# lukedan/libfluid

Hardware: AMD Instinct MI355X
Metric: particle_steps_per_sec (higher is better)
Workload: dtype f32

## Files before the change

### libfluid_amd/csrc/common.h

```cpp
#pragma once

#include <hip/hip_runtime.h>
#include <stdint.h>

#include <string>
#include <vector>

#include "../../include/libfluid_amd.h"
#include "slots.h"

hipError_t lfa_pool_malloc(void **p, size_t bytes);
hipError_t lfa_pool_free(void *p);
void lfa_pool_nosync_begin();
void lfa_pool_nosync_end();
template <typename T> inline hipError_t lfa_hip_malloc(T **p, size_t bytes) { return lfa_pool_malloc((void **)p, bytes); }
#define hipMalloc(p, n) lfa_hip_malloc((p), (n))
#define hipFree(p) lfa_pool_free((void *)(p))
struct lfa_stream_set;
lfa_stream_set *lfa_pool_take_set(int device);
void lfa_pool_park_set(lfa_stream_set *q);

#define LFA_TILE 8
#define LFA_TILE_CELLS 512
#define LFA_HALO 10
// ... 102 lines not shown
	float *uo = nullptr, *vo = nullptr, *wo = nullptr;
	uint8_t *ctype = nullptr, *solid = nullptr;
	uint32_t *cell_count = nullptr;
	uint32_t *fine_start = nullptr;
	float *stage = nullptr;
	size_t stage_tiles = 0;
	float *acc = nullptr;
	double bg[3] = {0, 0, 0};
	bool grid_valid = false;

	uint8_t *abits = nullptr;
	void *vp = nullptr, *vr = nullptr, *vz = nullptr, *vs = nullptr, *vpre = nullptr, *vq = nullptr;
	struct lfa_mg *mg = nullptr;
	int *nbr_table = nullptr;
	void *vs2 = nullptr;
	size_t vec_elem = 0;
	double *partials = nullptr;
	int *pcg_state = nullptr;
	double *pcg_hist = nullptr;
	int *level_tiles = nullptr;
	std::vector<int> level_offsets;
	GridDims g1{};
	size_t ncp1 = 0;
	float *c_diag = nullptr, *c_w[3] = {nullptr, nullptr, nullptr};
	uint8_t *c_unk = nullptr;
	void *c_pre = nullptr, *c_r = nullptr, *c_x = nullptr, *c_r2 = nullptr, *c_x2 = nullptr, *a2inv = nullptr;
	void *c_as = nullptr;
	int *slot_l1 = nullptr, *l1_tiles = nullptr, *l1_l2 = nullptr;
	int n_l1tiles = 0, n2 = 0, a2cap = 0;
	size_t coarse_elem = 0;
	double a_scale = 0.0, sys_dt = -1.0;
	uint64_t n_unknowns = 0;
	bool system_valid = false, unknown_count_valid = false;
	double last_residual = 0.0;
	uint64_t last_iters = 0;
	uint64_t stat_launches_iter = 0, stat_transport_iter = 0, stat_transport_solve = 0, stat_mg_levels = 0, stat_mg_first_co = 0;
	bool pcg_poisoned = false;
	bool last_rhs_zero = false;
	bool co_disabled = false;
	uint64_t stat_co_aborts = 0, stat_co_reason = 0;
	bool gate_counted = false;
	uint32_t *tile_epoch = nullptr;
	uint8_t *tile_closed = nullptr;
	uint32_t solve_epoch = 0;
	uint32_t pressure_epoch = 0;
	bool warm_started = false;
	uint32_t *vc_src = nullptr;
	size_t vc_extent = 0;
	bool vc_pending = false;
	uint64_t stat_p2g_deferred = 0;
	bool vmax2_valid = false;
	float *c_home = nullptr;
	size_t c_home_cap = 0;
	bool c_home_valid = false;
	bool vc_with_c = false;
	uint8_t *tile_clear = nullptr;
	unsigned clear_epoch = 0;
	unsigned solid_epoch = 1;

	struct SourceHost {
		std::vector<int32_t> xyz;
		double vel[3];
		uint64_t root;
		bool active, coerce;
		bool operator==(const SourceHost &o) const {
			return xyz == o.xyz && vel[0] == o.vel[0] && vel[1] == o.vel[1] && vel[2] == o.vel[2] && root == o.root &&
// ... 263 lines not shown
		v[k] = i < n ? p[i] : -INFINITY;
	}
	double a = -INFINITY;
#pragma unroll
	for (int k = 0; k < 8; ++k) {
		nan |= v[k] != v[k];
		a = v[k] > a ? v[k] : a;
	}
	for (int i = (int)threadIdx.x + 2048; i < n; i += 256) {
		const double x = p[i];
		nan |= x != x;
		a = x > a ? x : a;
	}
	return a;
}
template <typename T> __device__ inline T wave_sum(T v) {
#pragma unroll
	for (int o = 32; o > 0; o >>= 1) v += __shfl_xor(v, o, 64);
	return v;
}
template <typename T> __device__ inline T wave_max(T v) {
#pragma unroll
	for (int o = 32; o > 0; o >>= 1) {
		T other = __shfl_xor(v, o, 64);
		v = other > v ? other : v;
	}
	return v;
}

int lfa_exclusive_scan_u32(lfa_sim *s, const uint32_t *in, uint32_t *out, size_t n, uint32_t *total_dev);
int lfa_scan_total(lfa_sim *s, const uint32_t *in, uint32_t *out, size_t n, uint32_t *total_dev, int slot, size_t *total);

int lfa_particles_alloc(lfa_sim *s, size_t n);
int lfa_hash_particles_impl(lfa_sim *s, bool counts_done);
int lfa_particles_materialize(lfa_sim *s);
int lfa_c_home_restore(lfa_sim *s);
int lfa_c_home_ensure(lfa_sim *s, size_t n);
int lfa_ensure_io(lfa_sim *s, size_t bytes);
int lfa_slab_download_slots(lfa_sim *s, const uint32_t **slot);
int lfa_sample_velocity_launch(lfa_sim *s, hipStream_t stream, const double *xyz, size_t n, const uint32_t *tile_rule, int z_lo, int z_hi,
                               double *velocity, uint8_t *types, uint32_t *counts_dev);
int lfa_sample_refresh(lfa_sim *s, const char *who, size_t room_bytes, const uint32_t **tile_rule, void **room, int *z_lo, int *z_hi);
int lfa_pcg_alloc(lfa_sim *s);
int lfa_number_unknowns(lfa_sim *s);

__host__ __device__ inline int lfa_stage_index(int hx, int hy, int hz) {
	return (unsigned)(hx - 1) < 8u ? (hx - 1) + 8 * (hy + 10 * hz) : 800 + (hx ? 100 : 0) + hy + 10 * hz;
}
__host__ __device__ inline int lfa_stage_source(int o) {
	if (o < 800) return 1 + (o & 7) + 10 * (o >> 3);
	const int q = o - 800, pl = q >= 100 ? 1 : 0, r = q - 100 * pl;
	return 9 * pl + 10 * r;
}

struct lfa_dist {
	int rank = 0, nranks = 1;
	int device_share = 1;
	int exchange(lfa_sim *s, const void *send_lo, size_t n_send_lo, void *recv_lo, size_t n_recv_lo, const void *send_hi,
	             size_t n_send_hi, void *recv_hi, size_t n_recv_hi) {
		++calls;
		return exchange_impl(s, send_lo, n_send_lo, recv_lo, n_recv_lo, send_hi, n_send_hi, recv_hi, n_recv_hi);
	}
	int allreduce(lfa_sim *s, double *dev, int count, bool is_max) {
		++calls;
		return allreduce_impl(s, dev, count, is_max);
	}
	int allreduce_buf(lfa_sim *s, void *dev, size_t count, int dtype, bool is_max) {
// ... 44 lines not shown
```

### libfluid_amd/csrc/core.hip

```cpp
#include <math.h>

#include <algorithm>
#include <stdarg.h>
#include <stdio.h>
#include <string.h>

#include <mutex>

#include "common.h"
#include "pcg.h"
#include "stream_set.h"

static thread_local std::string g_create_error;

int lfa_fail(lfa_sim *s, int code, const char *fmt, ...) {
	char buf[512];
	va_list ap;
	va_start(ap, fmt);
	vsnprintf(buf, sizeof buf, fmt, ap);
	va_end(ap);
	if (s) s->err = buf;
	else g_create_error = buf;
	return code;
}
// ... 910 lines not shown
	pos_store(dst.pos, d, key, me.t[0], me.t[1], me.t[2]);
	bkey[d] = key;
	dst.id[d] = src.id[i];
	from[d] = (uint32_t)i;
}
__global__ void k_c_to_home(size_t n, ParticleSoA p, float *home, size_t stride) {
	size_t i = (size_t)blockIdx.x * blockDim.x + threadIdx.x;
	if (i >= n || p.pos[i].key == 0xFFFFFFFFu) return;
	const size_t j = p.id[i];
#pragma unroll
	for (int k = 0; k < 9; ++k) home[k * stride + j] = p.c[k][i];
}
__global__ void k_c_from_home(size_t n, ParticleSoA p, const float *home, size_t stride) {
	size_t i = (size_t)blockIdx.x * blockDim.x + threadIdx.x;
	if (i >= n || p.pos[i].key == 0xFFFFFFFFu) return;
	const size_t j = p.id[i];
#pragma unroll
	for (int k = 0; k < 9; ++k) p.c[k][i] = home[k * stride + j];
}
__global__ void k_gather_vc(size_t n, ParticleSoA old, ParticleSoA cur, const uint32_t *from, int with_c) {
	size_t d = (size_t)blockIdx.x * blockDim.x + threadIdx.x;
	if (d >= n) return;
	const uint32_t i = from[d];
#pragma unroll
	for (int k = 0; k < 3; ++k) cur.v[k][d] = old.v[k][i];
	if (with_c) {
#pragma unroll
		for (int k = 0; k < 9; ++k) cur.c[k][d] = old.c[k][i];
	}
}

#define CC_UNROLL 16
__global__ void __launch_bounds__(256)
k_cell_count(const int *dtiles, int n_dtiles, const uint32_t *key, const uint32_t *tile_start, uint32_t *cell_count) {
	__shared__ uint32_t cnt[LFA_TILE_CELLS];
	for (int slot = blockIdx.x; slot < n_dtiles; slot += gridDim.x) {
		int tile = dtiles[slot];
		cnt[threadIdx.x] = 0;
		cnt[threadIdx.x + 256] = 0;
		__syncthreads();
		uint32_t b = tile_start[tile], e = tile_start[tile + 1];
		for (uint32_t base = b + threadIdx.x; base - threadIdx.x < e; base += 256 * CC_UNROLL) {
			uint32_t k[CC_UNROLL];
#pragma unroll
			for (int q = 0; q < CC_UNROLL; ++q) {
				const uint32_t i = base + 256 * q;
				k[q] = key[i < e ? i : e - 1];
			}
#pragma unroll
			for (int q = 0; q < CC_UNROLL; ++q)
				if (base + 256 * q < e) atomicAdd(&cnt[k[q] & 511], 1u);
		}
		__syncthreads();
		cell_count[(size_t)tile * LFA_TILE_CELLS + threadIdx.x] = cnt[threadIdx.x];
		cell_count[(size_t)tile * LFA_TILE_CELLS + 256 + threadIdx.x] = cnt[threadIdx.x + 256];
		__syncthreads();
	}
}

__global__ void k_compact_range(const uint32_t *flag, const uint32_t *scan, int *list, int *slot_of, int lo, int hi,
                                int slot_base) {
	int t = lo + blockIdx.x * blockDim.x + threadIdx.x;
	if (t >= hi) return;
	if (flag[t]) {
		list[scan[t]] = t;
		if (slot_of) slot_of[t] = slot_base + (int)scan[t];
	} else if (slot_of) {
		slot_of[t] = -1;
	}
}
__global__ void k_fill_i32(int *p, int n, int v) {
	int i = blockIdx.x * blockDim.x + threadIdx.x;
	if (i < n) p[i] = v;
}
__global__ void k_gather_u32(const uint32_t *src, const int *idx, int n, uint32_t *dst) {
	int i = threadIdx.x;
	if (i < n) dst[i] = src[idx[i]];
}

__global__ void k_dilate_slots(const int *tile_pslot, uint32_t *flag, GridDims g) {
	const int t = blockIdx.x * blockDim.x + threadIdx.x;
	if (t >= g.nt || tile_pslot[t] < 0) return;
	int tx, ty, tz;
	tile_coords(g, t, tx, ty, tz);
	for (int o = 0; o < 27; ++o) {
		const int x = tx + o % 3 - 1, y = ty + (o / 3) % 3 - 1, z = tz + o / 9 - 1;
		if ((unsigned)x < (unsigned)g.ntx && (unsigned)y < (unsigned)g.nty && (unsigned)z < (unsigned)g.ntz)
			flag[x + g.ntx * (y + g.nty * z)] = 1u;
// ... 27 lines not shown
		const hipError_t e = hipStreamSynchronize(s->stream);
		if (e != hipSuccess) return fail(e, "hipStreamSynchronize");
		LFA_HIP(s, hipFree(s->c_home));
	}
	s->c_home = nh;
	s->c_home_cap = cap;
	return LFA_OK;
}
int lfa_c_home_restore(lfa_sim *s) {
	if (!s->c_home_valid) return LFA_OK;
	s->c_home_valid = false;
	const size_t n = s->binned ? s->np_live : s->np;
	if (!n) return LFA_OK;
	hipLaunchKernelGGL(k_c_from_home, dim3((unsigned)((n + 255) / 256)), dim3(256), 0, s->stream, n, s->pb[s->cur], (const float *)s->c_home,
	                   s->c_home_cap);
	LFA_LAUNCH_CHECK(s);
	return LFA_OK;
}

int lfa_particles_materialize(lfa_sim *s) {
	if (!s->vc_pending) return LFA_OK;
	LFA_TRY(lfa_corr_commit(s));
	s->vc_pending = false;
	LFA_HIP(s, hipSetDevice(s->device));
	const size_t n = s->np_live;
	if (!n) return LFA_OK;
	hipLaunchKernelGGL(k_gather_vc, dim3((unsigned)((n + 255) / 256)), dim3(256), 0, s->stream, n, s->pb[s->cur ^ 1], s->pb[s->cur],
	                   (const uint32_t *)s->vc_src, s->vc_with_c ? 1 : 0);
	LFA_LAUNCH_CHECK(s);
	return LFA_OK;
}

extern "C" int lfa_hash_particles(lfa_sim *s) { return lfa_hash_particles_impl(s, false); }
int lfa_hash_particles_impl(lfa_sim *s, bool counts_done) {
	if (!s) return LFA_E_INVALID;
	LFA_HIP(s, hipSetDevice(s->device));
	LFA_TRY(lfa_corr_commit(s));
	LFA_TRY(lfa_particles_materialize(s));
	const GridDims &g = s->g;
	const int nt = g.nt, L = g.ntx * g.nty;
	const size_t n = s->binned ? s->np_live : s->np;
	ParticleSoA &src = s->pb[s->cur], &dst = s->pb[s->cur ^ 1];
	const int own_lo = s->slab_lo * L, own_hi = s->slab_hi * L;
	const int all_lo = lfa_has_lo(s) ? own_lo - L : own_lo, all_hi = lfa_has_hi(s) ? own_hi + L : own_hi;

	if (!counts_done) {
		LFA_HIP(s, hipMemsetAsync(s->tile_count, 0, (size_t)(nt + 1) * 4, s->stream));
		if (n) {
			hipLaunchKernelGGL(k_tile_count, dim3((unsigned)((n + 256 * TC_CHUNKS - 1) / (256 * TC_CHUNKS))), dim3(256), 0, s->stream, (const PosRec *)src.pos, n,
			                   s->tile_count, s->rank);
			LFA_LAUNCH_CHECK(s);
		}
	}
	LFA_TRY(lfa_exclusive_scan_u32(s, s->tile_count, s->tile_start, (size_t)nt + 1, nullptr));
	LFA_HIP(s, hipMemcpyAsync(s->h_pinned + LFA_PIN_NP_LIVE, s->tile_start + nt, 4, hipMemcpyDeviceToHost, s->stream));

	hipLaunchKernelGGL(k_tile_flags, dim3((nt + 255) / 256), dim3(256), 0, s->stream, s->tile_count, s->tile_flag, nt);
	LFA_LAUNCH_CHECK(s);
	LFA_TRY(lfa_dist_exchange_tile_layers_u32(s, s->tile_flag));
	hipLaunchKernelGGL(k_fill_i32, dim3((nt + 255) / 256), dim3(256), 0, s->stream, s->tile_pslot, nt, -1);
	LFA_LAUNCH_CHECK(s);
	const bool one_sync = !s->dist;
	if (one_sync) {
		uint32_t *tot = (uint32_t *)s->pcg_state + LFA_DW_N_PTILES;
		LFA_TRY(compact_tiles_async(s, s->tile_flag, 0, nt, s->ptiles_all, s->tile_pslot, tot));
		LFA_HIP(s, hipMemsetAsync(s->tile_flag, 0, (size_t)(nt + 1) * 4, s->stream));
		hipLaunchKernelGGL(k_dilate_slots, dim3((nt + 255) / 256), dim3(256), 0, s->stream, (const int *)s->tile_pslot, s->tile_flag, g);
// ... 42 lines not shown
		s->n_ghost_lo = s->p_off;
		s->n_ghost_hi = s->n_ptiles_all - vals[3];
		s->ptiles = s->ptiles_all + s->p_off;
		s->n_dtiles = (int)h[LFA_SLAB_N_DTILES];
		for (int w = 0; w < 4; ++w) s->n_halo[w] = (int)h[LFA_SLAB_N_HALO + w];
	}
	s->np_live = s->h_pinned[LFA_PIN_NP_LIVE];
	if (s->dist) s->np = s->np_live;
	s->holes = false;
	s->n_arrivals = 0;
	s->move_pending = false;
	if (n) {
		const dim3 sgrid((unsigned)((n + 255) / 256));
		const bool home = s->prm.simulation_method != LFA_APIC;
		if (home && !s->c_home_valid) {
			LFA_TRY(lfa_c_home_ensure(s, s->dist ? std::max<size_t>(s->pcap, (size_t)s->next_global_id) : s->pcap));
			hipLaunchKernelGGL(k_c_to_home, sgrid, dim3(256), 0, s->stream, n, src, s->c_home, s->c_home_cap);
			LFA_LAUNCH_CHECK(s);
			s->c_home_valid = true;
		} else if (!home && s->c_home_valid) {
			LFA_TRY(lfa_c_home_restore(s));
		}
		hipLaunchKernelGGL(k_tile_scatter, sgrid, dim3(256), 0, s->stream, n, src, dst, s->rank, s->tile_start, s->tile_count,
		                   s->binned ? 0 : 1, s->vc_src, s->bkey);
		LFA_LAUNCH_CHECK(s);
		s->cur ^= 1;
		s->vc_pending = true;
		s->vc_extent = n;
		s->vc_with_c = !home;
	}
	if (s->n_dtiles) {
		int grid = s->n_dtiles < 8192 ? s->n_dtiles : 8192;
		hipLaunchKernelGGL(k_cell_count, dim3(grid), dim3(256), 0, s->stream, s->dtiles, s->n_dtiles,
		                   (const uint32_t *)s->bkey, s->tile_start, s->cell_count);
		LFA_LAUNCH_CHECK(s);
	}
	s->binned = true;
	s->system_valid = false;
	s->unknown_count_valid = false;
	return LFA_OK;
}

int lfa_dist_build_halo_lists(lfa_sim *s, const uint32_t *flag, int *lists, int n[4]) {
	const int L = s->g.ntx * s->g.nty;
	const int lo[4] = {s->slab_lo * L, (s->slab_hi - 1) * L, (s->slab_lo - 1) * L, s->slab_hi * L};
	const bool on[4] = {lfa_has_lo(s), lfa_has_hi(s), lfa_has_lo(s), lfa_has_hi(s)};
	uint32_t *tot = (uint32_t *)s->pcg_state + LFA_DW_SLAB + LFA_SLAB_N_HALO;
	LFA_HIP(s, hipMemsetAsync(tot, 0, 16, s->stream));
	for (int w = 0; w < 4; ++w)
		if (on[w]) LFA_TRY(compact_tiles_async(s, flag, lo[w], lo[w] + L, lists + (size_t)w * L, nullptr, tot + w));
	LFA_HIP(s, hipMemcpyAsync(s->h_pinned + LFA_PIN_SLAB + LFA_SLAB_N_HALO, tot, 16, hipMemcpyDeviceToHost, s->stream));
	LFA_HIP(s, hipStreamSynchronize(s->stream));
	for (int w = 0; w < 4; ++w) n[w] = (int)s->h_pinned[LFA_PIN_SLAB + LFA_SLAB_N_HALO + w];
	return LFA_OK;
}

__global__ void k_raw_unknown_flags(GridDims g, size_t nc, const uint32_t *cell_count, const uint32_t *tile_flag,
                                    uint32_t *flag, int z0, int z1) {
	size_t r = (size_t)blockIdx.x * blockDim.x + threadIdx.x;
	if (r >= nc) return;
	int x = (int)(r % g.nx), y = (int)((r / g.nx) % g.ny), z = (int)(r / ((size_t)g.nx * g.ny));
	uint32_t b = blocked_index(g, x, y, z);
	flag[r] = (z >= z0 && z < z1 && tile_flag[b >> 9] && cell_count[b] > 0) ? 1u : 0u;
}

int lfa_number_unknowns(lfa_sim *s) {
	if (s->unknown_count_valid) return LFA_OK;
	if (!s->binned) return lfa_fail(s, LFA_E_INVALID, "call lfa_hash_particles first");
	if (!s->raw_scan) LFA_HIP(s, hipMalloc(&s->raw_scan, (s->nc + 1) * 4));
// ... 243 lines not shown
```

### libfluid_amd/csrc/grid_ops.hip

```cpp
#include "common.h"
#include "pcg.h"

namespace {

struct GridView {
	GridDims g;
	const uint8_t *ctype, *solid;
	const uint32_t *cell_count, *tile_flag;
};
__device__ inline bool is_unknown_at(const GridView &gv, int x, int y, int z) {
	if (!in_grid(gv.g, x, y, z)) return false;
	uint32_t b = blocked_index(gv.g, x, y, z);
	return gv.tile_flag[b >> 9] && gv.cell_count[b] > 0;
}

#define HT_UNKNOWN 8
__device__ inline void stage_halo_types(const GridView &gv, int tx, int ty, int tz, uint8_t *H) {
	for (int i = threadIdx.x; i < LFA_HALO_CELLS; i += 256) {
		const int x = 8 * tx + i % 10 - 1, y = 8 * ty + (i / 10) % 10 - 1, z = 8 * tz + i / 100 - 1;
		uint8_t t = CT_SOLID;
		if (in_grid(gv.g, x, y, z)) {
			const uint32_t b = blocked_index(gv.g, x, y, z);
			if (gv.tile_flag[b >> 9]) t = (uint8_t)((gv.ctype[b] & 7) | (gv.cell_count[b] > 0 ? HT_UNKNOWN : 0));
			else t = gv.solid[b] ? CT_SOLID : CT_AIR;
// ... 447 lines not shown
		const float v2 = g2p_particle<METHOD>(
		    p, i, pold, (METHOD == LFA_FLIP_BLEND && from) ? from[i] : i, gp,
		    [&](int b0, int b1, int b2) { return make_int3(cx + b0, cy + b1, cz + b2); },
		    [&](int field, int comp, int3 c, int k) { return clamped_sample(g, F[field], comp, c.x + (k & 1), c.y + ((k >> 1) & 1), c.z + (k >> 2)); });
		vmax2 = fmaxf(vmax2, v2);
	}
	vmax2 = wave_max(vmax2);
	if ((threadIdx.x & 63) == 0 && vmax2 > 0.0f) atomicMax(vmax2_bits, __float_as_uint(vmax2));
}
}

static int grid_blocks(int n) { return n < 16384 ? (n > 0 ? n : 1) : 16384; }

int lfa_dist_refresh_grid(lfa_sim *s, bool with_topology) {
	if (!s->dist) return LFA_OK;
	void *f[9];
	int e[9], n = 0;
	f[n] = s->u; e[n++] = 4;
	f[n] = s->v; e[n++] = 4;
	f[n] = s->w; e[n++] = 4;
	if (with_topology) {
		f[n] = s->ctype; e[n++] = 1;
		f[n] = s->cell_count; e[n++] = 4;
		if (s->prm.simulation_method == LFA_FLIP_BLEND && s->uo) {
			f[n] = s->uo; e[n++] = 4;
			f[n] = s->vo; e[n++] = 4;
			f[n] = s->wo; e[n++] = 4;
		}
	}
	return lfa_dist_exchange_fields(s, n, f, e);
}
static GridView make_view(lfa_sim *s) { return GridView{s->g, s->ctype, s->solid, s->cell_count, s->tile_flag}; }

int lfa_build_rhs(lfa_sim *s, double dt) {
	if (!s->binned) return lfa_fail(s, LFA_E_INVALID, "lfa_build_system: call lfa_hash_particles first");
	LFA_TRY(lfa_pcg_alloc(s));
	LFA_TRY(lfa_dist_refresh_grid(s, true));
	s->a_scale = dt / (s->prm.density * s->prm.cell_size * s->prm.cell_size);
	s->sys_dt = dt;
	if (!s->n_ptiles) return LFA_OK;
	GridView gv = make_view(s);
	if (!s->tile_closed) {
		LFA_HIP(s, hipMalloc(&s->tile_closed, (size_t)s->g.nt));
		LFA_HIP(s, hipMemsetAsync(s->tile_closed, 0, (size_t)s->g.nt, s->stream));
	}
	hipLaunchKernelGGL(k_abits, dim3(grid_blocks(s->n_ptiles)), dim3(256), 0, s->stream, s->ptiles, s->n_ptiles, gv,
	                   s->abits, s->tile_closed);
	LFA_LAUNCH_CHECK(s);
	const int G = pcg_grid_uncapped(s->n_ptiles);
	const float inv_h = (float)(1.0 / s->prm.cell_size);
	if (!s->tile_epoch) {
		LFA_HIP(s, hipMalloc(&s->tile_epoch, (size_t)s->g.nt * 4));
		LFA_HIP(s, hipMemsetAsync(s->tile_epoch, 0, (size_t)s->g.nt * 4, s->stream));
	}
	s->warm_started = s->prm.pcg_warm_start && s->prm.precond != LFA_PRECOND_MIC0_EXACT && !s->dist && s->pressure_epoch == s->solve_epoch &&
	                  s->solve_epoch != 0;
	const uint32_t keep_epoch = s->warm_started ? s->solve_epoch : 0u;
	++s->solve_epoch;
	if (s->solve_epoch == 0) s->solve_epoch = 1;
	if (s->prm.pcg_dtype == LFA_PCG_F64)
		hipLaunchKernelGGL(k_rhs<double>, dim3(G), dim3(256), 0, s->stream, s->ptiles, s->n_ptiles, gv, s->u, s->v, s->w,
		                   (double *)s->vr, (double *)s->vp, inv_h, s->partials + PART_B2, s->tile_epoch, keep_epoch, s->solve_epoch);
	else
		hipLaunchKernelGGL(k_rhs<float>, dim3(G), dim3(256), 0, s->stream, s->ptiles, s->n_ptiles, gv, s->u, s->v, s->w,
		                   (float *)s->vr, (float *)s->vp, inv_h, s->partials + PART_B2, s->tile_epoch, keep_epoch, s->solve_epoch);
	LFA_LAUNCH_CHECK(s);
	return LFA_OK;
}

extern "C" int lfa_apply_pressure(lfa_sim *s, double dt) {
	if (!s) return LFA_E_INVALID;
	if (!s->binned || !s->vp) return lfa_fail(s, LFA_E_INVALID, "lfa_apply_pressure: no pressure on the device");
	LFA_HIP(s, hipSetDevice(s->device));
	if (s->dist) LFA_TRY(lfa_dist_exchange_slices(s, s->vp, s->prm.pcg_dtype == LFA_PCG_F64 ? 8 : 4));
	if (!s->n_dtiles) return LFA_OK;
	const float coeff = (float)(dt / (s->prm.density * s->prm.cell_size));
	GridView gv = make_view(s);
	dim3 grid(grid_blocks(s->n_dtiles));
	if (s->prm.pcg_dtype == LFA_PCG_F64)
		hipLaunchKernelGGL(k_apply_pressure<double>, grid, dim3(256), 0, s->stream, s->dtiles, s->n_dtiles, gv, s->u, s->v,
		                   s->w, (const double *)s->vp, coeff);
// ... 93 lines not shown
```

### libfluid_amd/csrc/mg.hip

```cpp
#include <mutex>

#include "pcg.h"

#include <limits.h>
#include <math.h>
#include <stdio.h>
#include <stdlib.h>

#include <algorithm>
#include <vector>

#define MG_MAX_LEVELS 12
#define MG_NBR_STRIDE 8
#ifndef MG_INNER_SWEEPS
#define MG_INNER_SWEEPS 2
#endif
#define MG_OMEGA 1.15

struct lfa_mg_level {
	GridDims g{};
	size_t ncp = 0;
	int n_tiles = 0;
	int *tiles = nullptr;
	int *nbr = nullptr;
// ... 2269 lines not shown
	}
	size_t wgs;
	LFA_TRY(mg_co_capacity<real>(s, false, 0, &wgs));
	auto fits = [&](int first, bool tg) {
		const int nlev = last - first + 1;
		if (nlev > MG_CO_MAX_LEVELS || mg_co_capacity<real>(s, tg, nlev, &wgs) != LFA_OK) return false;
		const size_t share = s->dist ? (size_t)std::max(1, s->dist->device_share) : 1;
		return M.lv[first].n_tiles <= MG_CO_MAX_TILES && (size_t)M.lv[first].n_tiles * share <= wgs;
	};
	auto first_inside = [&](bool tg) {
		int tl = last;
		while (tl > 1 && tl - 1 >= D && fits(tl - 1, tg)) --tl;
		return std::max(tl, std::max(D, 1));
	};
	bool tagged = sizeof(real) == 4 && !s->knobs.mg_no_tagged;
	int tail = first_inside(tagged);
	if (tagged) {
		for (int l = tail; l <= last && tagged; ++l) tagged = mg_ensure_xq(s, M.lv[l], 3);
		if (!tagged) tail = first_inside(false);
	}
	P.tail = tail;
	P.tagged = tagged;
	const bool shared_gpu = s->dist && s->dist->device_share > 1;
	if (tagged && !shared_gpu && tail - 1 >= std::max(D, 1) && M.lv[tail - 1].n_tiles > 0 && !s->knobs.mg_no_top &&
	    M.lv[tail - 1].n_tiles <= MG_TOP_MAX_TILES && mg_ensure_xq(s, M.lv[tail - 1], 1))
		P.top = tail - 1;
	return LFA_OK;
}

static int mg_plan(lfa_sim *s);

template <typename real> static int mg_setup_t(lfa_sim *s) {
	if (!s->mg) s->mg = new lfa_mg();
	MgSetup U;
	LFA_TRY(mg_setup_levels<real>(s, U));
	if (U.D) LFA_TRY(mg_setup_host_lists(s, U));
	else LFA_TRY(mg_setup_device_lists<real>(s, U));
	LFA_TRY(mg_setup_operators<real>(s, U));
	LFA_TRY(mg_setup_exchange_abits(s, U));
	return mg_plan(s);
}

int lfa_mg_setup(lfa_sim *s) {
	return s->prm.pcg_dtype == LFA_PCG_F64 ? mg_setup_t<double>(s) : mg_setup_t<float>(s);
}

template <typename real> static MgLv<real> mg_lv(const lfa_sim *s, int l) {
	const lfa_mg_level &L = s->mg->lv[l];
	return MgLv<real>{L.tiles, L.nbr, L.n_tiles, L.g, l == 0 ? (const uint8_t *)s->abits : (const uint8_t *)L.abits,
	                  l == 0 ? (real *)s->vr : (real *)L.b, l == 0 ? (real *)s->vq : (real *)L.x, l == 0 ? (real *)s->vz : (real *)L.y};
}

template <typename real> static int mg_launch_coarse(lfa_sim *s, int top, void (*co_kernel)(MgCo<real>, const int *)) {
	lfa_mg &M = *s->mg;
	const MgPlan &P = M.plan;
	const int last = P.last, tail = P.tail;
	const int *st = (const int *)s->pcg_state;
	if (P.persist) {
		MgCo<real> C;
		C.first = tail;
		C.last = last;
		C.nsw = MG_COARSEST_SWEEPS;
		C.inner = MG_INNER_SWEEPS;
		for (int l = tail; l <= last; ++l) {
			C.lv[l] = mg_lv<real>(s, l);
			C.ready[l] = M.lv[l].ready;
// ... 295 lines not shown
```

### libfluid_amd/csrc/p2g.hip

```cpp
#include "common.h"

namespace {

__device__ inline void axis_bf(float t, bool own, int &b, float &f) {
	if (own) {
		b = t >= 1.0f ? 0 : -1;
		f = t >= 1.0f ? 0.0f : t;
	} else {
		b = t < 0.5f ? -1 : 0;
		f = t < 0.5f ? t + 0.5f : t - 0.5f;
	}
}

template <bool APIC, bool QUIRK, typename AddFn>
__device__ inline void scatter_particle(int lx, int ly, int lz, const float t[3], const float v[3], const float c[9],
                                        float hworld, int rot, AddFn add) {
	if (QUIRK) {
#pragma unroll
		for (int comp = 0; comp < 3; ++comp) {
			float w1[3][3], a1[3][3];
			const float *cc = c + 3 * comp;
#pragma unroll
			for (int a = 0; a < 3; ++a)
#pragma unroll
// ... 171 lines not shown
}

template <bool APIC, bool QUIRK>
__global__ void __launch_bounds__(256)
k_p2g_atomic(size_t n, ParticleSoA p, float *acc, size_t ncp, GridDims g, float hworld) {
	size_t i = (size_t)blockIdx.x * blockDim.x + threadIdx.x;
	if (i >= n) return;
	const PosRec me = pos_load(p.pos, i);
	const uint32_t key = me.key;
	const int tile = (int)(key >> 9), l = (int)(key & 511);
	int tx, ty, tz;
	tile_coords(g, tile, tx, ty, tz);
	const int cx = tx * 8 + (l & 7), cy = ty * 8 + ((l >> 3) & 7), cz = tz * 8 + (l >> 6);
	float t[3] = {me.t[0], me.t[1], me.t[2]};
	float v[3] = {p.v[0][i], p.v[1][i], p.v[2][i]};
	float c[9];
	if (APIC) {
#pragma unroll
		for (int k = 0; k < 9; ++k) c[k] = p.c[k][i];
	}
	scatter_particle<APIC, QUIRK>(0, 0, 0, t, v, c, hworld, 0, [&](int comp, int hx, int hy, int hz, float wv, float wgt) {
		int x = cx + hx - 1, y = cy + hy - 1, z = cz + hz - 1;
		if (!in_grid(g, x, y, z)) return;
		size_t b = blocked_index(g, x, y, z);
		unsafeAtomicAdd(acc + (size_t)(2 * comp) * ncp + b, wv);
		unsafeAtomicAdd(acc + (size_t)(2 * comp + 1) * ncp + b, wgt);
	});
}

struct FinalizeParams {
	int method;
	float g[3];
	int fuse_gravity;
};

template <bool BINNED>
__global__ void __launch_bounds__(256)
k_p2g_finalize(const int *dtiles, int n_dtiles, GridDims g, const int *tile_pslot, const float *stage, const float *acc,
               size_t ncp, const uint32_t *cell_count, const uint8_t *solid, float *u, float *v, float *w, float *uo,
               float *vo, float *wo, uint8_t *ctype, FinalizeParams fp) {
	__shared__ int ps27[27];
	for (int slot = blockIdx.x; slot < n_dtiles; slot += gridDim.x) {
		const int tile = dtiles[slot];
		int tx, ty, tz;
		tile_coords(g, tile, tx, ty, tz);
		if (BINNED) {
			__syncthreads();
			if (threadIdx.x < 27) {
				const int nx_ = tx + (int)threadIdx.x % 3 - 1, ny_ = ty + ((int)threadIdx.x / 3) % 3 - 1, nz_ = tz + (int)threadIdx.x / 9 - 1;
				const bool in = (unsigned)nx_ < (unsigned)g.ntx && (unsigned)ny_ < (unsigned)g.nty && (unsigned)nz_ < (unsigned)g.ntz;
				ps27[threadIdx.x] = in ? tile_pslot[nx_ + g.ntx * (ny_ + g.nty * nz_)] : -1;
			}
			__syncthreads();
		}
#pragma unroll
		for (int half = 0; half < 2; ++half) {
			const int l = threadIdx.x + 256 * half;
			const int lx = l & 7, ly = (l >> 3) & 7, lz = l >> 6;
			const size_t b = (size_t)tile * LFA_TILE_CELLS + l;
			const int x = tx * 8 + lx, y = ty * 8 + ly, z = tz * 8 + lz;
			float s[6] = {0.f, 0.f, 0.f, 0.f, 0.f, 0.f};
			if (BINNED) {
				const int ox0 = lx == 0 ? -1 : 0, ox1 = lx == 7 ? 1 : 0, oy0 = ly == 0 ? -1 : 0, oy1 = ly == 7 ? 1 : 0;
				const int oz0 = lz == 0 ? -1 : 0, oz1 = lz == 7 ? 1 : 0;
				for (int oz = oz0; oz <= oz1; ++oz)
					for (int oy = oy0; oy <= oy1; ++oy)
						for (int ox = ox0; ox <= ox1; ++ox) {
							const int ps = ps27[(ox + 1) + 3 * (oy + 1) + 9 * (oz + 1)];
							if (ps < 0) continue;
							const float *src = stage + (size_t)ps * 6 * LFA_HALO_CELLS + lfa_stage_index(lx - 8 * ox + 1, ly - 8 * oy + 1, lz - 8 * oz + 1);
#pragma unroll
							for (int k = 0; k < 6; ++k) s[k] += src[k * LFA_HALO_CELLS];
						}
			} else {
#pragma unroll
				for (int k = 0; k < 6; ++k) s[k] = acc[(size_t)k * ncp + b];
			}
			const bool inside = in_grid(g, x, y, z);
			float vel[3];
#pragma unroll
			for (int k = 0; k < 3; ++k) vel[k] = s[2 * k + 1] > 1e-6f ? s[2 * k] / s[2 * k + 1] : 0.0f;
			uint8_t type;
			if (!inside) {
				vel[0] = vel[1] = vel[2] = 0.0f;
				type = CT_SOLID | CT_OUTSIDE;
			} else if (solid[b]) {
				type = CT_SOLID;
			} else {
				type = cell_count[b] > 0 ? CT_FLUID : CT_AIR;
			}
			const bool bx = x == g.nx - 1, by = y == g.ny - 1, bz = z == g.nz - 1;
			if (fp.method == LFA_FLIP_BLEND && inside) {
				uo[b] = bx ? 0.0f : vel[0];
				vo[b] = by ? 0.0f : vel[1];
				wo[b] = bz ? 0.0f : vel[2];
			}
			if (fp.method == LFA_APIC) {
				if (bx) vel[0] = 0.0f;
				if (by) vel[1] = 0.0f;
				if (bz) vel[2] = 0.0f;
			}
			if (fp.fuse_gravity && inside) {
				vel[0] += fp.g[0]; vel[1] += fp.g[1]; vel[2] += fp.g[2];
			}
			u[b] = vel[0]; v[b] = vel[1]; w[b] = vel[2];
			ctype[b] = type;
		}
	}
}

__global__ void __launch_bounds__(256)
k_add_gravity(const int *dtiles, int n_dtiles, GridDims g, float *u, float *v, float *w, float gx, float gy, float gz) {
	for (int slot = blockIdx.x; slot < n_dtiles; slot += gridDim.x) {
		const int tile = dtiles[slot];
		int tx, ty, tz;
		tile_coords(g, tile, tx, ty, tz);
#pragma unroll
		for (int half = 0; half < 2; ++half) {
			const int l = threadIdx.x + 256 * half;
			if (!in_grid(g, tx * 8 + (l & 7), ty * 8 + ((l >> 3) & 7), tz * 8 + (l >> 6))) continue;
			const size_t b = (size_t)tile * LFA_TILE_CELLS + l;
			u[b] += gx; v[b] += gy; w[b] += gz;
		}
	}
}
}

static int grid_blocks(int n) { return n < 16384 ? (n > 0 ? n : 1) : 16384; }

static int scatter_mode(const lfa_sim *s) {
	if (s->prm.simulation_method != LFA_APIC) return 0;
	return (s->prm.apic_unscaled_kernel && s->prm.cell_size != 1.0) ? 2 : 1;
}
static void launch_binned(lfa_sim *s, const ParticleSoA &p, const ParticleSoA &pvc, const uint32_t *from, float *stage_own) {
	const dim3 grid(grid_blocks(s->n_ptiles));
	const float hworld = (float)s->prm.cell_size;
#define LB(A, Q)                                                                                                             \
	hipLaunchKernelGGL((k_p2g_binned<A, Q>), grid, dim3(P2G_THREADS), 0, s->stream, s->ptiles, s->n_ptiles, p, pvc, from, s->tile_start, \
	                   stage_own, hworld, rot_mask)
// ... 41 lines not shown
			s->stage = nullptr;
			size_t want = (size_t)s->n_ptiles_all + (size_t)s->n_ptiles_all / 4 + 16;
			hipError_t e = hipMalloc(&s->stage, want * 6 * LFA_HALO_CELLS * 4);
			if (e != hipSuccess) return lfa_fail(s, LFA_E_OOM, "hipMalloc of the P2G staging slabs (%zu tiles) failed", want);
			s->stage_tiles = want;
		}
		if (s->n_ptiles) {
			launch_binned(s, p, pvc, from, s->stage + (size_t)s->p_off * 6 * LFA_HALO_CELLS);
			LFA_LAUNCH_CHECK(s);
			if (from) ++s->stat_p2g_deferred;
		}
		LFA_TRY(lfa_dist_exchange_p2g_planes(s, s->stage));
	} else {
		if (s->dist) return lfa_fail(s, LFA_E_UNSUPPORTED, "the global-atomic P2G variant is single-GPU only");
		if (!s->acc) {
			hipError_t e = hipMalloc(&s->acc, s->ncp * 6 * 4);
			if (e != hipSuccess) return lfa_fail(s, LFA_E_OOM, "hipMalloc of the atomic P2G accumulators failed");
		}
		if (s->n_dtiles) {
			hipLaunchKernelGGL(k_zero_acc, dim3(s->n_dtiles), dim3(256), 0, s->stream, s->dtiles, s->n_dtiles, s->acc,
			                   s->ncp);
			LFA_LAUNCH_CHECK(s);
		}
		if (s->np_live) {
			launch_atomic(s, p);
			LFA_LAUNCH_CHECK(s);
		}
	}
	LFA_TRY(lfa_ev_record(s, LFA_EV_SCATTER_END));
	FinalizeParams fp;
	fp.method = method;
	fp.fuse_gravity = fuse_gravity ? 1 : 0;
	for (int k = 0; k < 3; ++k) fp.g[k] = fuse_gravity ? (float)(s->prm.gravity[k] * dt) : 0.0f;
	if (s->n_dtiles) {
		dim3 grid(grid_blocks(s->n_dtiles));
		if (binned)
			hipLaunchKernelGGL(k_p2g_finalize<true>, grid, dim3(256), 0, s->stream, s->dtiles, s->n_dtiles, s->g,
			                   s->tile_pslot, s->stage, s->acc, s->ncp, s->cell_count, s->solid, s->u, s->v, s->w, s->uo,
			                   s->vo, s->wo, s->ctype, fp);
		else
			hipLaunchKernelGGL(k_p2g_finalize<false>, grid, dim3(256), 0, s->stream, s->dtiles, s->n_dtiles, s->g,
			                   s->tile_pslot, s->stage, s->acc, s->ncp, s->cell_count, s->solid, s->u, s->v, s->w, s->uo,
			                   s->vo, s->wo, s->ctype, fp);
		LFA_LAUNCH_CHECK(s);
	}
	LFA_HIP(s, hipMemcpyAsync(s->grid_flag, s->tile_flag, (size_t)s->g.nt * 4, hipMemcpyDeviceToDevice, s->stream));
	s->grid_valid = true;
	s->system_valid = false;
	for (int k = 0; k < 3; ++k) s->bg[k] = fuse_gravity ? s->prm.gravity[k] * dt : 0.0;
	return LFA_OK;
}

extern "C" int lfa_p2g(lfa_sim *s) {
	if (!s) return LFA_E_INVALID;
	return lfa_p2g_run(s, false, 0.0);
}

extern "C" int lfa_add_gravity(lfa_sim *s, double dt) {
	if (!s) return LFA_E_INVALID;
	LFA_HIP(s, hipSetDevice(s->device));
	if (s->binned && s->n_dtiles) {
		hipLaunchKernelGGL(k_add_gravity, dim3(grid_blocks(s->n_dtiles)), dim3(256), 0, s->stream, s->dtiles, s->n_dtiles,
		                   s->g, s->u, s->v, s->w, (float)(s->prm.gravity[0] * dt), (float)(s->prm.gravity[1] * dt),
		                   (float)(s->prm.gravity[2] * dt));
		LFA_LAUNCH_CHECK(s);
	}
	for (int k = 0; k < 3; ++k) s->bg[k] += s->prm.gravity[k] * dt;
	s->system_valid = false;
	return LFA_OK;
}

int lfa_p2g_bench(lfa_sim *s, int which) {
	if (which == LFA_K_P2G_SCATTER && s->prm.p2g_variant != LFA_P2G_LDS_BINNED) LFA_TRY(lfa_particles_materialize(s));
	const ParticleSoA &p = s->pb[s->cur], &pvc = s->vc_pending ? s->pb[s->cur ^ 1] : s->pb[s->cur];
	const uint32_t *from = s->vc_pending ? (const uint32_t *)s->vc_src : (const uint32_t *)nullptr;
	if (which == LFA_K_P2G_SCATTER) {
		if (s->prm.p2g_variant == LFA_P2G_LDS_BINNED) {
			if (!s->stage || (size_t)s->n_ptiles_all > s->stage_tiles) return lfa_fail(s, LFA_E_INVALID, "no staging slabs");
			launch_binned(s, p, pvc, from, s->stage + (size_t)s->p_off * 6 * LFA_HALO_CELLS);
		} else {
			if (!s->acc) return lfa_fail(s, LFA_E_INVALID, "no accumulators");
			launch_atomic(s, p);
		}
		LFA_LAUNCH_CHECK(s);
		return LFA_OK;
	}
	if (which == LFA_K_P2G_FINALIZE) {
		FinalizeParams fp;
		fp.method = s->prm.simulation_method;
		fp.fuse_gravity = 0;
		fp.g[0] = fp.g[1] = fp.g[2] = 0.f;
		dim3 grid(grid_blocks(s->n_dtiles));
		if (s->prm.p2g_variant == LFA_P2G_LDS_BINNED)
			hipLaunchKernelGGL(k_p2g_finalize<true>, grid, dim3(256), 0, s->stream, s->dtiles, s->n_dtiles, s->g,
			                   s->tile_pslot, s->stage, s->acc, s->ncp, s->cell_count, s->solid, s->u, s->v, s->w, s->uo,
			                   s->vo, s->wo, s->ctype, fp);
		else
			hipLaunchKernelGGL(k_p2g_finalize<false>, grid, dim3(256), 0, s->stream, s->dtiles, s->n_dtiles, s->g,
			                   s->tile_pslot, s->stage, s->acc, s->ncp, s->cell_count, s->solid, s->u, s->v, s->w, s->uo,
			                   s->vo, s->wo, s->ctype, fp);
		LFA_LAUNCH_CHECK(s);
		return LFA_OK;
	}
	if (which == LFA_K_BIN) return lfa_hash_particles(s);
	return lfa_fail(s, LFA_E_INVALID, "unknown kernel id %d", which);
}
```

### libfluid_amd/csrc/particles.hip

```cpp
#include <math.h>

#include <algorithm>
#include <utility>

#include "common.h"
#include "pcg.h"

namespace {

__device__ inline bool solid_or_outside(const GridDims &g, const uint8_t *solid, int x, int y, int z) {
	if (!in_grid(g, x, y, z)) return true;
	return solid[blocked_index(g, x, y, z)] != 0;
}

__device__ inline void collide(const GridDims &g, const uint8_t *solid, double from[3], double to[3], double skin) {
	for (int bounce = 0; bounce < 3; ++bounce) {
		bool hit = false;
		double diff[3], inv[3], t[3];
		int cur[3], last[3], adv[3];
#pragma unroll
		for (int d = 0; d < 3; ++d) {
			cur[d] = (int)floor(from[d]);
			last[d] = (int)floor(to[d]);
			diff[d] = to[d] - from[d];
// ... 1517 lines not shown
}
}

extern "C" int lfa_correct_collide_undo(lfa_sim *s) {
	if (!s) return LFA_E_INVALID;
	if (!s->corr_begun) return LFA_OK;
	if (!s->corr_undo_valid)
		return lfa_fail(s, LFA_E_INVALID, "lfa_correct_collide_undo: positions, binning or solid cells have changed since lfa_correct_collide_begin");
	LFA_HIP(s, hipSetDevice(s->device));
	LFA_TRY(lfa_corr_commit(s));
	s->corr_begun = false;
	const size_t n = s->np_live;
	if (!n) return LFA_OK;
	ParticleSoA &cur = s->pb[s->cur];
	hipLaunchKernelGGL(k_correct_undo, dim3((unsigned)((n + 255) / 256)), dim3(256), 0, s->stream, n, (const float4 *)correction_scratch(s),
	                   (const uint32_t *)s->bkey, cur.pos);
	LFA_LAUNCH_CHECK(s);
	return LFA_OK;
}

int lfa_g2p_stale(lfa_sim *s);
extern "C" int lfa_time_step(lfa_sim *s, double dt, double *residual, uint64_t *iterations) {
	if (!s) return LFA_E_INVALID;
	if (s->src_rng_on && s->dist && !(s->src_rng_flags & LFA_SEED_COLLECTIVE))
		return lfa_fail(s, LFA_E_UNSUPPORTED, "lfa_time_step: fluid sources that draw from the pcg32 (lfa_set_source_rng) on a slab decomposition");
	LFA_HIP(s, hipSetDevice(s->device));
	LFA_TRY(lfa_corr_commit(s));
	LFA_TRY(lfa_ev_record(s, LFA_EV_STEP_START));
	LFA_TRY(advect_collide(s, dt, true));
	LFA_TRY(lfa_ev_record(s, LFA_EV_STEP_ADVECT));
	{
		const bool counted = s->counts_fresh;
		s->counts_fresh = false;
		LFA_TRY(lfa_hash_particles_impl(s, counted));
	}
	if (!s->sources.empty()) LFA_TRY(lfa_update_sources(s, nullptr));
	LFA_TRY(lfa_ev_record(s, LFA_EV_STEP_BIN));
	const bool overlap = s->overlap_correction && (s->dist || s->np_live);
	LFA_TRY(lfa_p2g_run(s, true, dt));
	LFA_TRY(lfa_ev_record(s, LFA_EV_STEP_P2G));
	if (overlap) {
		if (s->dist) LFA_TRY(lfa_dist_exchange_ghost_particles(s));
		LFA_TRY(correct_begin(s, dt, true));
	}
	double res = 0.0;
	uint64_t it = 0;
	int rc = LFA_OK;
	auto grid_stages = [&]() -> int {
		rc = lfa_pcg_solve(s, dt, &res, &it);
		if (rc < 0) return rc;
		LFA_TRY(lfa_ev_record(s, LFA_EV_STEP_SOLVE));
		LFA_TRY(lfa_apply_pressure(s, dt));
		LFA_TRY(lfa_ev_record(s, LFA_EV_STEP_APPLY));
		if (!overlap) {
			LFA_TRY(lfa_correct_collide(s, dt));
			LFA_TRY(lfa_ev_record(s, LFA_EV_STEP_CORRECT));
		}
		LFA_TRY(lfa_extrapolate(s));
		return lfa_ev_record(s, LFA_EV_STEP_EXTRAP);
	};
	const int rc_grid = grid_stages();
	if (overlap) LFA_TRY(lfa_corr_join(s));
	if (rc_grid < 0) return rc_grid;
	if (overlap && s->dist) LFA_TRY(lfa_dist_migrate(s, true));
	LFA_TRY(lfa_ev_record(s, LFA_EV_STEP_JOIN));
	LFA_TRY(lfa_g2p_stale(s));
	if (s->timing) {
// ... 80 lines not shown
```

### libfluid_amd/csrc/pcg.h

```cpp
#pragma once
#include "common.h"

#define PCG_MAX_GRID 2048
#define PCG_WAVES 4
enum { PART_STRIDE = PCG_MAX_GRID + 64, PART_ZS = 0, PART_RMAX = PART_STRIDE, PART_SIG0 = 2 * PART_STRIDE,
       PART_SIG1 = 3 * PART_STRIDE, PART_B2 = 4 * PART_STRIDE, PART_TOTAL = 5 * PART_STRIDE };

extern int lfa_pcg_grid_cap;
static inline int pcg_grid(int n_ptiles) {
	int g = (n_ptiles + PCG_WAVES - 1) / PCG_WAVES;
	if (g < 1) g = 1;
	return g < lfa_pcg_grid_cap ? g : lfa_pcg_grid_cap;
}

static inline int pcg_grid_uncapped(int n_ptiles) {
	int g = (n_ptiles + PCG_WAVES - 1) / PCG_WAVES;
	if (g < 1) g = 1;
	return g < PCG_MAX_GRID ? g : PCG_MAX_GRID;
}

#define halo_at(x, y, z) (((x) + 1) + 10 * ((y) + 1) + 100 * ((z) + 1))
#define store_halo_faces(h, lx, ly, v) \
	do {                               \
		(h)[halo_at(-1, lx, ly)] = (v)[0]; \
// ... 11 lines not shown
	                        (size_t)7 * 64 + lane, (size_t)lane};
	real v[6];
#pragma unroll
	for (int k = 0; k < 6; ++k) v[k] = nb[k] >= 0 ? ld((size_t)nb[k] * 512 + cell[k]) : (real)0;
	store_halo_faces(h, lx, ly, v);
}
template <typename real> __device__ inline real stencil_row(const real *H, uint32_t a, int i) {
	const real F = (a & AB_FLUID) ? (real)1 : (real)0;
	real val = (real)(a & 7) * H[i];
	val = madd01(-F, H[i - 1], val);
	val = madd01(-F, H[i - 10], val);
	val = madd01(-F, H[i - 100], val);
	val = madd01(-(real)((a >> 3) & 1), H[i + 1], val);
	val = madd01(-(real)((a >> 4) & 1), H[i + 10], val);
	val = madd01(-(real)((a >> 5) & 1), H[i + 100], val);
	return val;
}
template <typename real> __device__ inline real residual_cell(const real *H, uint32_t a, real b, int i) {
	real r = (real)0;
	if (a & AB_UNKNOWN) r = b - stencil_row<real>(H, a, i);
	return r;
}
__device__ inline double nan_max(double x, double y) { return (x != x || y != y) ? NAN : (y > x ? y : x); }
__device__ inline bool verdict_stops(double rmax, double tol) { return rmax != rmax || rmax < tol; }
__device__ inline void record_verdict(int *state, double *hist, int slot, double rmax, bool stops) {
	hist[slot] = rmax;
	if (stops) {
		if (rmax != rmax) state[LFA_DW_NAN] = 1;
		*(double *)(state + LFA_DW_RESIDUAL) = rmax;
		state[LFA_DW_DONE] = slot + 1;
	}
}

int lfa_build_rhs(lfa_sim *s, double dt);
int lfa_p2g_run(lfa_sim *s, bool fuse_gravity, double dt);
int lfa_dist_refresh_grid(lfa_sim *s, bool with_topology);

int lfa_mg_setup(lfa_sim *s);
int lfa_mg_apply(lfa_sim *s, double *part_sigma);
struct lfa_mg_stop {
	const double *part_rmax = nullptr;
	int n_part = 0, iter = 0;
};
template <typename real>
int lfa_mg_axpy_apply(lfa_sim *s, const void *sdir, const double *part_sigma, int n_sigma, const double *part_qs, int n_qs,
                      double *part_rmax, double *part_sigma_new, const lfa_mg_stop &stop);
template <typename real>
int lfa_mg_axpy_apply_cg(lfa_sim *s, const double *gamma, int n_gamma, const double *gamma_old, int n_gamma_old, const double *delta,
                         int n_delta, const double *rmax_prev, int n_rmax, int iter, double *alpha_io, double *part_rmax,
                         double *part_sigma_new);
int lfa_mg_bench_part(lfa_sim *s, int part);
int lfa_mg_level0(const lfa_sim *s, const int **tiles, const int **slot);
int lfa_mg_solve_closed(lfa_sim *s, void *out = nullptr);
void lfa_mg_free(lfa_sim *s);
void lfa_mg_stats(const lfa_sim *s, uint64_t *launches_per_cycle, uint64_t *levels, uint64_t *first_co);
```

### libfluid_amd/csrc/pcg.hip

```cpp
#include "pcg.h"

#include <math.h>
#include <string.h>

#include <stdlib.h>

#include <algorithm>

namespace {

#define WAVE_SYNC() asm volatile("s_waitcnt lgkmcnt(0)" ::: "memory")

template <typename real> struct Vecs {
	real *p, *r, *z, *s, *pre, *q;
};

struct TileCtx {
	const int *ptiles;
	int n_ptiles;
	const int *tile_pslot;
	GridDims g;
};

__device__ inline void face_neighbours(const TileCtx &tc, int tile, int nb[6]) {
// ... 1427 lines not shown
	} else {
		const bool embed = is_ml(s) && r1_ready && s->n_l1tiles <= 64;
		if (embed) {
			hipLaunchKernelGGL((k_mic_apply<real, SWEEP_BOTH, true>), dim3(G + PCG_COARSE_BLOCKS), dim3(256), 0, s->stream, tc,
			                   (const int *)nullptr, s->n_ptiles, s->abits, v, scale, part_sigma, s->pcg_state, (real *)nullptr,
			                   (const int *)s->slot_l1, make_coarse<real>(s, (real *)s->c_r), embedded_coarse(s));
			LFA_LAUNCH_CHECK(s);
		} else {
			hipLaunchKernelGGL((k_mic_apply<real, SWEEP_BOTH, false>), dim3(G), dim3(256), 0, s->stream, tc,
			                   (const int *)nullptr, s->n_ptiles, s->abits, v, scale, part_sigma, s->pcg_state,
			                   (is_ml(s) && !r1_ready) ? (real *)s->c_r : (real *)nullptr, (const int *)s->slot_l1,
			                   CoarseFields<real>{}, CoarseArgs{});
			LFA_LAUNCH_CHECK(s);
			if (is_ml(s)) LFA_TRY(coarse_apply<real>(s, (real *)s->c_r, part_sigma, s->stream));
		}
	}
	return LFA_OK;
}

static int pcg_scrub(lfa_sim *s) {
	LFA_HIP(s, hipStreamSynchronize(s->stream));
	lfa_mg_free(s);
	void *vs[] = {s->vp, s->vr, s->vz, s->vs, s->vpre, s->vq, s->vs2};
	for (void *v : vs)
		if (v) LFA_HIP(s, hipMemsetAsync(v, 0, s->ncp * s->vec_elem, s->stream));
	s->pressure_epoch = 0;
	s->warm_started = false;
	s->pcg_poisoned = false;
	return LFA_OK;
}

template <typename real> static int build_system_t(lfa_sim *s, double dt) {
	if (s->pcg_poisoned) LFA_TRY(pcg_scrub(s));
	LFA_TRY(lfa_build_rhs(s, dt));
	if (s->n_ptiles || (s->dist && is_mg(s))) LFA_TRY(mic_factor<real>(s));
	s->system_valid = true;
	return LFA_OK;
}

extern "C" int lfa_build_system(lfa_sim *s, double dt) {
	if (!s) return LFA_E_INVALID;
	LFA_HIP(s, hipSetDevice(s->device));
	LFA_TRY(lfa_pcg_alloc(s));
	return s->prm.pcg_dtype == LFA_PCG_F64 ? build_system_t<double>(s, dt) : build_system_t<float>(s, dt);
}

template <typename real, typename... Args>
static void launch_pcg_a(bool first, bool coarse, int grid, hipStream_t st, Args... a) {
	if (first && coarse) hipLaunchKernelGGL((k_pcg_a<real, true, true>), dim3(grid), dim3(256), 0, st, a...);
	else if (first) hipLaunchKernelGGL((k_pcg_a<real, true, false>), dim3(grid), dim3(256), 0, st, a...);
	else if (coarse) hipLaunchKernelGGL((k_pcg_a<real, false, true>), dim3(grid), dim3(256), 0, st, a...);
	else hipLaunchKernelGGL((k_pcg_a<real, false, false>), dim3(grid), dim3(256), 0, st, a...);
}
template <typename real>
static void launch_pcg_b(lfa_sim *s, bool embed, int grid, const real *s_cur, const double *sig, int n_sig, const double *zs, int n_zs,
                         double *sig_new, real *cr_cur, real *cr_next) {
	const Vecs<real> v = make_vecs<real>(s);
	const real scale = (real)s->a_scale;
	double *rmax = s->partials + PART_RMAX;
	if (embed) {
		CoarseFields<real> cf = make_coarse<real>(s, cr_cur);
		cf.as = (const real *)s->c_as;
		hipLaunchKernelGGL((k_pcg_b<real, true>), dim3(grid + PCG_COARSE_BLOCKS), dim3(256), 0, s->stream, (const int *)s->ptiles,
		                   s->n_ptiles, s->abits, v, s_cur, scale, sig, n_sig, zs, n_zs, rmax, sig_new, s->pcg_state, cr_next,
		                   (const int *)s->slot_l1, cf, embedded_coarse(s));
	} else {
// ... 566 lines not shown
```

Baseline: 5.647 billion.

## Compute cell types during cell counting and split abits from RHS build

Cell type classification (outside/solid/fluid/air) moves into the k_cell_count kernel during particle hashing, so the P2G finalize kernel can skip recomputing and storing ctype when the counts and solid epoch are still current. lfa_build_rhs is split into lfa_build_abits and a separate RHS build, which makes it possible to schedule the two independently. The change also resets the multigrid closed_out flag on setup. It adds a dependency on epoch tracking to decide whether types are stale, which risks stale types if solids change without an epoch bump.

After: 5.646 billion. No clear change (-0.0%).

```diff
diff --git a/libfluid_amd/csrc/common.h b/libfluid_amd/csrc/common.h
--- a/libfluid_amd/csrc/common.h
+++ b/libfluid_amd/csrc/common.h
@@ -158,6 +158,8 @@
 	double a_scale = 0.0, sys_dt = -1.0;
 	uint64_t n_unknowns = 0;
 	bool system_valid = false, unknown_count_valid = false;
+	bool types_from_count = false;
+	unsigned types_solid_epoch = 0;
 	double last_residual = 0.0;
 	uint64_t last_iters = 0;
 	uint64_t stat_launches_iter = 0, stat_transport_iter = 0, stat_transport_solve = 0, stat_mg_levels = 0, stat_mg_first_co = 0;
@@ -487,7 +489,7 @@
 int lfa_scan_total(lfa_sim *s, const uint32_t *in, uint32_t *out, size_t n, uint32_t *total_dev, int slot, size_t *total);
 
 int lfa_particles_alloc(lfa_sim *s, size_t n);
-int lfa_hash_particles_impl(lfa_sim *s, bool counts_done);
+int lfa_hash_particles_impl(lfa_sim *s, bool counts_done, bool with_types = false);
 int lfa_particles_materialize(lfa_sim *s);
 int lfa_c_home_restore(lfa_sim *s);
 int lfa_c_home_ensure(lfa_sim *s, size_t n);
diff --git a/libfluid_amd/csrc/core.hip b/libfluid_amd/csrc/core.hip
--- a/libfluid_amd/csrc/core.hip
+++ b/libfluid_amd/csrc/core.hip
@@ -966,7 +966,8 @@
 
 #define CC_UNROLL 16
 __global__ void __launch_bounds__(256)
-k_cell_count(const int *dtiles, int n_dtiles, const uint32_t *key, const uint32_t *tile_start, uint32_t *cell_count) {
+k_cell_count(const int *dtiles, int n_dtiles, const uint32_t *key, const uint32_t *tile_start, uint32_t *cell_count, GridDims g,
+             const uint8_t *solid, uint8_t *ctype) {
 	__shared__ uint32_t cnt[LFA_TILE_CELLS];
 	for (int slot = blockIdx.x; slot < n_dtiles; slot += gridDim.x) {
 		int tile = dtiles[slot];
@@ -988,6 +989,20 @@
 		__syncthreads();
 		cell_count[(size_t)tile * LFA_TILE_CELLS + threadIdx.x] = cnt[threadIdx.x];
 		cell_count[(size_t)tile * LFA_TILE_CELLS + 256 + threadIdx.x] = cnt[threadIdx.x + 256];
+		if (ctype) {
+			int tx, ty, tz;
+			tile_coords(g, tile, tx, ty, tz);
+#pragma unroll
+			for (int half = 0; half < 2; ++half) {
+				const int l = (int)threadIdx.x + 256 * half;
+				const size_t cell = (size_t)tile * LFA_TILE_CELLS + l;
+				uint8_t type;
+				if (!in_grid(g, tx * 8 + (l & 7), ty * 8 + ((l >> 3) & 7), tz * 8 + (l >> 6))) type = CT_SOLID | CT_OUTSIDE;
+				else if (solid[cell]) type = CT_SOLID;
+				else type = cnt[l] > 0 ? CT_FLUID : CT_AIR;
+				ctype[cell] = type;
+			}
+		}
 		__syncthreads();
 	}
 }
@@ -1081,7 +1096,7 @@
 }
 
 extern "C" int lfa_hash_particles(lfa_sim *s) { return lfa_hash_particles_impl(s, false); }
-int lfa_hash_particles_impl(lfa_sim *s, bool counts_done) {
+int lfa_hash_particles_impl(lfa_sim *s, bool counts_done, bool with_types) {
 	if (!s) return LFA_E_INVALID;
 	LFA_HIP(s, hipSetDevice(s->device));
 	LFA_TRY(lfa_corr_commit(s));
@@ -1190,9 +1205,12 @@
 	if (s->n_dtiles) {
 		int grid = s->n_dtiles < 8192 ? s->n_dtiles : 8192;
 		hipLaunchKernelGGL(k_cell_count, dim3(grid), dim3(256), 0, s->stream, s->dtiles, s->n_dtiles,
-		                   (const uint32_t *)s->bkey, s->tile_start, s->cell_count);
+		                   (const uint32_t *)s->bkey, s->tile_start, s->cell_count, s->g, (const uint8_t *)s->solid,
+		                   with_types ? s->ctype : (uint8_t *)nullptr);
 		LFA_LAUNCH_CHECK(s);
 	}
+	s->types_from_count = with_types;
+	s->types_solid_epoch = s->solid_epoch;
 	s->binned = true;
 	s->system_valid = false;
 	s->unknown_count_valid = false;
diff --git a/libfluid_amd/csrc/grid_ops.hip b/libfluid_amd/csrc/grid_ops.hip
--- a/libfluid_amd/csrc/grid_ops.hip
+++ b/libfluid_amd/csrc/grid_ops.hip
@@ -503,7 +503,7 @@
 }
 static GridView make_view(lfa_sim *s) { return GridView{s->g, s->ctype, s->solid, s->cell_count, s->tile_flag}; }
 
-int lfa_build_rhs(lfa_sim *s, double dt) {
+int lfa_build_abits(lfa_sim *s, double dt) {
 	if (!s->binned) return lfa_fail(s, LFA_E_INVALID, "lfa_build_system: call lfa_hash_particles first");
 	LFA_TRY(lfa_pcg_alloc(s));
 	LFA_TRY(lfa_dist_refresh_grid(s, true));
@@ -518,6 +518,14 @@
 	hipLaunchKernelGGL(k_abits, dim3(grid_blocks(s->n_ptiles)), dim3(256), 0, s->stream, s->ptiles, s->n_ptiles, gv,
 	                   s->abits, s->tile_closed);
 	LFA_LAUNCH_CHECK(s);
+	return LFA_OK;
+}
+
+int lfa_build_rhs(lfa_sim *s, double dt) {
+	s->a_scale = dt / (s->prm.density * s->prm.cell_size * s->prm.cell_size);
+	s->sys_dt = dt;
+	if (!s->n_ptiles) return LFA_OK;
+	GridView gv = make_view(s);
 	const int G = pcg_grid_uncapped(s->n_ptiles);
 	const float inv_h = (float)(1.0 / s->prm.cell_size);
 	if (!s->tile_epoch) {
diff --git a/libfluid_amd/csrc/mg.hip b/libfluid_amd/csrc/mg.hip
--- a/libfluid_amd/csrc/mg.hip
+++ b/libfluid_amd/csrc/mg.hip
@@ -2325,6 +2325,7 @@
 
 template <typename real> static int mg_setup_t(lfa_sim *s) {
 	if (!s->mg) s->mg = new lfa_mg();
+	s->mg->closed_out = false;
 	MgSetup U;
 	LFA_TRY(mg_setup_levels<real>(s, U));
 	if (U.D) LFA_TRY(mg_setup_host_lists(s, U));
diff --git a/libfluid_amd/csrc/p2g.hip b/libfluid_amd/csrc/p2g.hip
--- a/libfluid_amd/csrc/p2g.hip
+++ b/libfluid_amd/csrc/p2g.hip
@@ -227,6 +227,7 @@
 	int method;
 	float g[3];
 	int fuse_gravity;
+	int store_types;
 };
 
 template <bool BINNED>
@@ -275,14 +276,13 @@
 			float vel[3];
 #pragma unroll
 			for (int k = 0; k < 3; ++k) vel[k] = s[2 * k + 1] > 1e-6f ? s[2 * k] / s[2 * k + 1] : 0.0f;
-			uint8_t type;
-			if (!inside) {
-				vel[0] = vel[1] = vel[2] = 0.0f;
-				type = CT_SOLID | CT_OUTSIDE;
-			} else if (solid[b]) {
-				type = CT_SOLID;
-			} else {
-				type = cell_count[b] > 0 ? CT_FLUID : CT_AIR;
+			if (!inside) vel[0] = vel[1] = vel[2] = 0.0f;
+			if (fp.store_types) {
+				uint8_t type;
+				if (!inside) type = CT_SOLID | CT_OUTSIDE;
+				else if (solid[b]) type = CT_SOLID;
+				else type = cell_count[b] > 0 ? CT_FLUID : CT_AIR;
+				ctype[b] = type;
 			}
 			const bool bx = x == g.nx - 1, by = y == g.ny - 1, bz = z == g.nz - 1;
 			if (fp.method == LFA_FLIP_BLEND && inside) {
@@ -299,7 +299,6 @@
 				vel[0] += fp.g[0]; vel[1] += fp.g[1]; vel[2] += fp.g[2];
 			}
 			u[b] = vel[0]; v[b] = vel[1]; w[b] = vel[2];
-			ctype[b] = type;
 		}
 	}
 }
@@ -407,6 +406,8 @@
 	fp.method = method;
 	fp.fuse_gravity = fuse_gravity ? 1 : 0;
 	for (int k = 0; k < 3; ++k) fp.g[k] = fuse_gravity ? (float)(s->prm.gravity[k] * dt) : 0.0f;
+	const bool types_done = binned && s->types_from_count && s->types_solid_epoch == s->solid_epoch;
+	fp.store_types = types_done ? 0 : 1;
 	if (s->n_dtiles) {
 		dim3 grid(grid_blocks(s->n_dtiles));
 		if (binned)
@@ -464,6 +465,7 @@
 		FinalizeParams fp;
 		fp.method = s->prm.simulation_method;
 		fp.fuse_gravity = 0;
+		fp.store_types = 1;
 		fp.g[0] = fp.g[1] = fp.g[2] = 0.f;
 		dim3 grid(grid_blocks(s->n_dtiles));
 		if (s->prm.p2g_variant == LFA_P2G_LDS_BINNED)
diff --git a/libfluid_amd/csrc/particles.hip b/libfluid_amd/csrc/particles.hip
--- a/libfluid_amd/csrc/particles.hip
+++ b/libfluid_amd/csrc/particles.hip
@@ -1573,7 +1573,7 @@
 	{
 		const bool counted = s->counts_fresh;
 		s->counts_fresh = false;
-		LFA_TRY(lfa_hash_particles_impl(s, counted));
+		LFA_TRY(lfa_hash_particles_impl(s, counted, !s->dist));
 	}
 	if (!s->sources.empty()) LFA_TRY(lfa_update_sources(s, nullptr));
 	LFA_TRY(lfa_ev_record(s, LFA_EV_STEP_BIN));
diff --git a/libfluid_amd/csrc/pcg.h b/libfluid_amd/csrc/pcg.h
--- a/libfluid_amd/csrc/pcg.h
+++ b/libfluid_amd/csrc/pcg.h
@@ -67,6 +67,7 @@
 	}
 }
 
+int lfa_build_abits(lfa_sim *s, double dt);
 int lfa_build_rhs(lfa_sim *s, double dt);
 int lfa_p2g_run(lfa_sim *s, bool fuse_gravity, double dt);
 int lfa_dist_refresh_grid(lfa_sim *s, bool with_topology);
diff --git a/libfluid_amd/csrc/pcg.hip b/libfluid_amd/csrc/pcg.hip
--- a/libfluid_amd/csrc/pcg.hip
+++ b/libfluid_amd/csrc/pcg.hip
@@ -1483,6 +1483,7 @@
 
 template <typename real> static int build_system_t(lfa_sim *s, double dt) {
 	if (s->pcg_poisoned) LFA_TRY(pcg_scrub(s));
+	LFA_TRY(lfa_build_abits(s, dt));
 	LFA_TRY(lfa_build_rhs(s, dt));
 	if (s->n_ptiles || (s->dist && is_mg(s))) LFA_TRY(mic_factor<real>(s));
 	s->system_valid = true;
```
